# liruiw/OMG-Planner

Measured on AMD Instinct MI355X. Metric: CHOMP iterations/sec (batched scenes) + ms/plan, Panda 7-DoF 30-wp, higher is better.
Workload: dtype f32 SDF / f64 kinematics+update; 1 GPU; 100 table-top scenes/GPU x (64-goal goal-set cost + CHOMP step), Panda 9-dof, 30 waypoints; scenes_per_gpu=100, total_scenes=100, goals=64, waypoints=30, sdf_grid=4x64^3 + 128x96x32 per scene, private, goal_selection=MD on device (omgx_goal_update_optimize), pipeline_parts=3, top_k_collision=1000, plan_restart_every_steps=50

## Files before the change

### omg-planner_amd/csrc/omg_device.h

```cpp
#pragma once
#include <hip/hip_runtime.h>
#include <stdint.h>

#include "../../include/omg_hip.h"

#define OMG_WAVE 64

namespace omg {

struct __attribute__((packed, aligned(4))) F2 { float a, b; };
struct __attribute__((packed, aligned(4))) F4 { float a, b, c, d; };

__device__ __forceinline__ float lerpf(float a, float b, float t) { return __builtin_fmaf(t, b - a, a); }

struct Axis { int i0; float f; bool ok; };
__device__ __forceinline__ Axis axis_of(float g) {
    Axis a;
    a.ok = (g > -1.0e9f) && (g <= 1.0e9f);
    const float s = g - 0.5f;
    a.i0 = (int)s;
    a.f = s - (float)a.i0;
    const bool edge = (s == -1.0f) && (g > -0.5f);
    a.i0 = edge ? 0 : a.i0;
    a.f = edge ? -1.0f : a.f;
// ... 21 lines not shown
    const bool in = ax.ok && ay.ok && az.ok && ax.i0 >= 0 && ax.i0 < G.dx - 1 && ay.i0 >= 0 && ay.i0 < G.dy - 1 &&
                    az.i0 >= 0 && az.i0 < G.dz - 1;
    if (!in) return 1.0f;
    const int b = G.idx(ax.i0, ay.i0, az.i0);
    const int sy = G.dz, sx = G.dy * G.dz;
    const F2 r00 = *reinterpret_cast<const F2*>(G.g + b);
    const F2 r01 = *reinterpret_cast<const F2*>(G.g + b + sy);
    const F2 r10 = *reinterpret_cast<const F2*>(G.g + b + sx);
    const F2 r11 = *reinterpret_cast<const F2*>(G.g + b + sx + sy);
    return trilerp(r00.a, r00.b, r01.a, r01.b, r10.a, r10.b, r11.a, r11.b, ax.f, ay.f, az.f);
}

struct ObjParams {
    float T[12];
    float lo[3], hi[3];
    int dim[3];
    float delta, eps, pad, clr;
    double rw[3];
    float rc[3], rh[3], rr2;
    double rdelta;
    float i2eps, ieps;
};

__device__ __forceinline__ bool rbox_inside(float tx, float ty, float tz, const float* c, const float* h, float r2) {
    const float dx = __builtin_fmaxf(__builtin_fabsf(tx - c[0]) - h[0], 0.0f);
    const float dy = __builtin_fmaxf(__builtin_fabsf(ty - c[1]) - h[1], 0.0f);
    const float dz = __builtin_fmaxf(__builtin_fabsf(tz - c[2]) - h[2], 0.0f);
    return __builtin_fmaf(dz, dz, __builtin_fmaf(dy, dy, dx * dx)) <= r2;
}
__device__ __forceinline__ bool rbox_near(float ux, float uy, float uz, float rad, const float* c, const float* h, float r) {
    const float dx = __builtin_fmaxf(__builtin_fabsf(ux - c[0]) - h[0], 0.0f);
    const float dy = __builtin_fmaxf(__builtin_fabsf(uy - c[1]) - h[1], 0.0f);
    const float dz = __builtin_fmaxf(__builtin_fabsf(uz - c[2]) - h[2], 0.0f);
    const float rr = r + rad;
    return __builtin_fmaf(dz, dz, __builtin_fmaf(dy, dy, dx * dx)) <= rr * rr * 1.000001f;
}

__device__ __forceinline__ void derive_far_box(ObjParams& o) {
#pragma unroll
    for (int k = 0; k < 3; ++k) {
        const float w = o.hi[k] - o.lo[k];
        const bool ok = w > 0.0f && o.dim[k] > 0;
        const float vox = w / (float)(o.dim[k] > 0 ? o.dim[k] : 1);
        o.rc[k] = ok ? 0.5f * w : 0.0f;
        o.rh[k] = ok ? 0.5f * w + 1.5f * vox : __builtin_inff();
    }
    o.rr2 = 0.0f;
    o.rdelta = 1.0 / (double)o.delta;
    o.i2eps = 1.0f / (2.0f * o.eps);
    o.ieps = 1.0f / o.eps;
}

struct Accum { float pot, gx, gy, gz, col; };

struct PairPrep { float tx, ty, tz; bool far; };

__device__ __forceinline__ PairPrep pair_prepare(const ObjParams& o, float px, float py, float pz) {
    const float* T = o.T;
    const float ux = __builtin_fmaf(T[2], pz, __builtin_fmaf(T[1], py, __builtin_fmaf(T[0], px, T[3])));
    const float uy = __builtin_fmaf(T[6], pz, __builtin_fmaf(T[5], py, __builtin_fmaf(T[4], px, T[7])));
    const float uz = __builtin_fmaf(T[10], pz, __builtin_fmaf(T[9], py, __builtin_fmaf(T[8], px, T[11])));
    PairPrep r;
    r.tx = ux - o.lo[0]; r.ty = uy - o.lo[1]; r.tz = uz - o.lo[2];
    const bool inside = rbox_inside(r.tx, r.ty, r.tz, o.rc, o.rh, o.rr2);
    r.far = (o.eps < 1.0f && o.clr <= 1.0f) ? !inside : false;
    return r;
}

template <bool WANT_GRAD>
__device__ __forceinline__ void pair_exact(const ObjParams& o, const float* __restrict__ grid, float tx, float ty, float tz,
                                           Accum& acc) {
    const float* T = o.T;
    const float gx = (float)((double)tx * o.rw[0]) * (float)o.dim[0];
    const float gy = (float)((double)ty * o.rw[1]) * (float)o.dim[1];
    const float gz = (float)((double)tz * o.rw[2]) * (float)o.dim[2];
    Grid G{grid, o.dim[0], o.dim[1], o.dim[2]};
    const Axis ax = axis_of(gx), ay = axis_of(gy), az = axis_of(gz);
    const bool in_c = ax.ok && ay.ok && az.ok && ax.i0 >= 0 && ax.i0 < G.dx - 1 && ay.i0 >= 0 && ay.i0 < G.dy - 1 &&
                      az.i0 >= 0 && az.i0 < G.dz - 1;
    if (!in_c) {
        if (1.0f < o.clr) acc.col += 1.0f;
        if (!(1.0f <= o.eps)) return;
    }
    const int sy = G.dz, sx = G.dy * G.dz;
    const int b = G.idx(ax.i0, ay.i0, az.i0);

    if (!WANT_GRAD) {
        const int bb = in_c ? b : 0;
        const F2 r00 = *reinterpret_cast<const F2*>(G.g + bb);
        const F2 r01 = *reinterpret_cast<const F2*>(G.g + bb + sy);
        const F2 r10 = *reinterpret_cast<const F2*>(G.g + bb + sx);
        const F2 r11 = *reinterpret_cast<const F2*>(G.g + bb + sx + sy);
        const float tv = trilerp(r00.a, r00.b, r01.a, r01.b, r10.a, r10.b, r11.a, r11.b, ax.f, ay.f, az.f);
        const float value = in_c ? tv : 1.0f;
        acc.col += (in_c && value < o.clr) ? 1.0f : 0.0f;
        const float p_in = (float)(-(double)value + 0.5 * (double)o.eps);
        const float d = value - o.eps;
        const float p_band = o.i2eps * d * d * o.pad;
        acc.pot += value <= 0.0f ? p_in : (value <= o.eps ? p_band : 0.0f);
        return;
    }

    const Axis axp = axis_of(gx + 1.0f), axm = axis_of(gx - 1.0f);
    const Axis ayp = axis_of(gy + 1.0f), aym = axis_of(gy - 1.0f);
    const Axis azp = axis_of(gz + 1.0f), azm = axis_of(gz - 1.0f);
    const bool regular = axp.i0 == ax.i0 + 1 && axm.i0 == ax.i0 - 1 && ayp.i0 == ay.i0 + 1 && aym.i0 == ay.i0 - 1 &&
                         azp.i0 == az.i0 + 1 && azm.i0 == az.i0 - 1 && axp.ok && axm.ok && ayp.ok && aym.ok && azp.ok && azm.ok;
    const bool interior = in_c && regular && ax.i0 >= 1 && ax.i0 < G.dx - 2 && ay.i0 >= 1 && ay.i0 < G.dy - 2 &&
                          az.i0 >= 1 && az.i0 < G.dz - 2;

    float value, fpx, fmx, fpy, fmy, fpz, fmz;
    if (interior) {
        const F4 c00 = *reinterpret_cast<const F4*>(G.g + b - 1);
        const F4 c01 = *reinterpret_cast<const F4*>(G.g + b + sy - 1);
        const F4 c10 = *reinterpret_cast<const F4*>(G.g + b + sx - 1);
        const F4 c11 = *reinterpret_cast<const F4*>(G.g + b + sx + sy - 1);
        value = trilerp(c00.b, c00.c, c01.b, c01.c, c10.b, c10.c, c11.b, c11.c, ax.f, ay.f, az.f);
        if (value < o.clr) acc.col += 1.0f;
        if (!(value <= 0.0f || value <= o.eps)) return;
        fpz = trilerp(c00.c, c00.d, c01.c, c01.d, c10.c, c10.d, c11.c, c11.d, ax.f, ay.f, azp.f);
        fmz = trilerp(c00.a, c00.b, c01.a, c01.b, c10.a, c10.b, c11.a, c11.b, ax.f, ay.f, azm.f);
        const F2 xp0 = *reinterpret_cast<const F2*>(G.g + b + 2 * sx);
        const F2 xp1 = *reinterpret_cast<const F2*>(G.g + b + 2 * sx + sy);
        const F2 xm0 = *reinterpret_cast<const F2*>(G.g + b - sx);
        const F2 xm1 = *reinterpret_cast<const F2*>(G.g + b - sx + sy);
        fpx = trilerp(c10.b, c10.c, c11.b, c11.c, xp0.a, xp0.b, xp1.a, xp1.b, axp.f, ay.f, az.f);
        fmx = trilerp(xm0.a, xm0.b, xm1.a, xm1.b, c00.b, c00.c, c01.b, c01.c, axm.f, ay.f, az.f);
        const F2 yp0 = *reinterpret_cast<const F2*>(G.g + b + 2 * sy);
        const F2 yp1 = *reinterpret_cast<const F2*>(G.g + b + sx + 2 * sy);
        const F2 ym0 = *reinterpret_cast<const F2*>(G.g + b - sy);
        const F2 ym1 = *reinterpret_cast<const F2*>(G.g + b + sx - sy);
        fpy = trilerp(c01.b, c01.c, yp0.a, yp0.b, c11.b, c11.c, yp1.a, yp1.b, ax.f, ayp.f, az.f);
        fmy = trilerp(ym0.a, ym0.b, c00.b, c00.c, ym1.a, ym1.b, c10.b, c10.c, ax.f, aym.f, az.f);
    } else {
        if (in_c) {
            value = sdf_value(G, ax, ay, az);
            if (value < o.clr) acc.col += 1.0f;
            if (!(value <= 0.0f || value <= o.eps)) return;
        } else {
            value = 1.0f;
        }
        fpx = sdf_value(G, axp, ay, az);
        fpy = sdf_value(G, ax, ayp, az);
        fpz = sdf_value(G, ax, ay, azp);
        fmx = sdf_value(G, axm, ay, az);
        fmy = sdf_value(G, ax, aym, az);
        fmz = sdf_value(G, ax, ay, azm);
    }
    const float g0 = (float)(0.5 * (double)(fpx - fmx) * o.rdelta);
    const float g1 = (float)(0.5 * (double)(fpy - fmy) * o.rdelta);
    const float g2 = (float)(0.5 * (double)(fpz - fmz) * o.rdelta);
    float v0, v1, v2;
    if (value <= 0.0f) {
        acc.pot += (float)(-(double)value + 0.5 * (double)o.eps);
        v0 = -g0; v1 = -g1; v2 = -g2;
    } else {
        const float d = value - o.eps;
        acc.pot += o.i2eps * d * d * o.pad;
        const float ie = o.ieps;
        v0 = ie * g0 * d * o.pad; v1 = ie * g1 * d * o.pad; v2 = ie * g2 * d * o.pad;
    }
    acc.gx += __builtin_fmaf(T[8], v2, __builtin_fmaf(T[4], v1, T[0] * v0));
    acc.gy += __builtin_fmaf(T[9], v2, __builtin_fmaf(T[5], v1, T[1] * v0));
    acc.gz += __builtin_fmaf(T[10], v2, __builtin_fmaf(T[6], v1, T[2] * v0));
}

template <bool WANT_GRAD>
__device__ __forceinline__ void sdf_pair(const ObjParams& o, const float* __restrict__ grid, float px, float py, float pz,
                                         Accum& acc) {
    const PairPrep pp = pair_prepare(o, px, py, pz);
    if (!pp.far) pair_exact<WANT_GRAD>(o, grid, pp.tx, pp.ty, pp.tz, acc);
}

#define OMG_CONST_AS __attribute__((address_space(4)))
typedef const OMG_CONST_AS omgx_object* ObjTablePtr;
typedef const OMG_CONST_AS int32_t* IntTablePtr;
#define OMG_GLOBAL_AS __attribute__((address_space(1)))
typedef const OMG_GLOBAL_AS char* GlobalBytes;
typedef float F2v __attribute__((ext_vector_type(2), aligned(4)));
__device__ __forceinline__ F2 global_f2(GlobalBytes p) { const F2v v = *(const OMG_GLOBAL_AS F2v*)p; return F2{v.x, v.y}; }
__device__ __forceinline__ ObjTablePtr as_const(const omgx_object* p) { return (ObjTablePtr)(uintptr_t)p; }
__device__ __forceinline__ IntTablePtr as_const(const int32_t* p) { return (IntTablePtr)(uintptr_t)p; }

__device__ __forceinline__ ObjParams load_object(ObjTablePtr ob) {
    ObjParams o;
#pragma unroll
    for (int k = 0; k < 12; ++k) o.T[k] = ob->pose_inv[k];
#pragma unroll
    for (int k = 0; k < 3; ++k) { o.lo[k] = ob->lo[k]; o.hi[k] = ob->hi[k]; o.dim[k] = ob->dim[k]; }
// ... 290 lines not shown
```

### omg-planner_amd/csrc/omg_goalset_queue.h

```cpp
#pragma once

#define GQ_TBL_MAX 32
#ifndef GQ_WG_PER_CU
#define GQ_WG_PER_CU 5
#endif
#ifndef GQ_WAVES
#define GQ_WAVES 4
#endif
#define GQ_NT (64 * GQ_WAVES)

struct GqFar {
    float T[12], lo[3], rc[3], rh[3], rr2, rb_r;
    bool cullable;
    int disabled;
};

typedef uint32_t GqU16 __attribute__((ext_vector_type(16)));
typedef uint32_t GqU8 __attribute__((ext_vector_type(8)));
typedef uint32_t GqU4 __attribute__((ext_vector_type(4)));
static_assert(offsetof(omgx_object, pose_inv) == 0 && offsetof(omgx_object, lo) == 0x30 && offsetof(omgx_object, epsilon) == 0x58 &&
              offsetof(omgx_object, clearance) == 0x60 && offsetof(omgx_object, disabled) == 0x64 && offsetof(omgx_object, rb_c) == 0x88 &&
              offsetof(omgx_object, rb_h) == 0x94 && offsetof(omgx_object, rb_r) == 0xa0 && offsetof(omgx_object, rb_r2) == 0xa4 &&
              sizeof(omgx_object) >= 0xa8, "gq_load_far reads the record by byte offsets");
__device__ __forceinline__ GqFar gq_load_far(ObjTablePtr ob) {
// ... 66 lines not shown
}
__device__ __forceinline__ void gq_tbl_store(uint32_t* e, const GqTblRec& r) {
#pragma unroll
    for (int k = 0; k < 3; ++k) {
        e[2 * k] = (uint32_t)__double2loint(r.rw[k]); e[2 * k + 1] = (uint32_t)__double2hiint(r.rw[k]);
        e[6 + k] = (uint32_t)r.dim[k];
    }
    e[9] = (uint32_t)(r.goffb & 0xffffffffll); e[10] = (uint32_t)(r.goffb >> 32);
    e[11] = __float_as_uint(0.5f * r.eps);
    e[12] = __float_as_uint(r.eps); e[13] = __float_as_uint(r.clr);
    e[14] = __float_as_uint(r.pad); e[15] = __float_as_uint(r.i2e);
}

template <bool PERSIST>
__device__ __forceinline__ double gq_ld_traj(const double* p) {
    if constexpr (PERSIST) return __hip_atomic_load(p, __ATOMIC_RELAXED, __HIP_MEMORY_SCOPE_AGENT);
    else return *p;
}
template <bool PERSIST>
__device__ __forceinline__ void gq_st_out(float* p, float v) {
    if constexpr (PERSIST) __hip_atomic_store(p, v, __ATOMIC_RELAXED, __HIP_MEMORY_SCOPE_AGENT);
    else *p = v;
}

template <int LB, bool STAMP, bool LAT, bool SPLIT, bool PRE, bool PERSIST = false, int ROLE = 0, int W = GQ_WAVES, bool RANGE = false>
__device__ __forceinline__ void gq_item(const ChunkArgs& a, double* const lds_pose, const int s, const bool is_layer, const int layer_part, const int chunk, const int NP) {
    const int o_begin = as_const(a.scene_begin)[s], o_end = as_const(a.scene_begin)[s + 1];
    const int P = a.P;
    const bool warming = LAT && o_end > o_begin;
    const int goal = NP > 1 ? chunk / NP : chunk;
    const int part = NP > 1 ? chunk - goal * NP : 0;
    static_assert(!RANGE || (SPLIT && !LAT && !PRE && !PERSIST && W == GQ_WAVES), "waypoint ranges: the batch kernel with two parts per goal and their own kinematics");
    const int CHg = a.CH;
    const int cfg_off = (RANGE && part > 0) ? a.range_h : 0;
    const int CH = RANGE ? (part > 0 ? CHg - a.range_h : a.range_h) : CHg;
    const int blk_shift = (4 - (CH & 3)) & 3;
    const int p = threadIdx.x & 15, lane = threadIdx.x & 63;
    const int wave = __builtin_amdgcn_readfirstlane((int)(threadIdx.x >> 6));
    const int tid = (int)threadIdx.x;
    const RobotViewS rv(a.robot, P);
    const int pstride = a.PS, MR = a.MR;
    static_assert(W == GQ_WAVES || (!LAT && !SPLIT && !PRE && !PERSIST && W >= 4), "wide workgroups: the batch kernel with whole goals and its own kinematics");
    constexpr int NT = 64 * W;
    const GqLayout L(pstride, MR, P, a.tbl_n, LAT, W);
    char* const lds_bytes = reinterpret_cast<char*>(lds_pose);
    uint32_t* const rowmask = reinterpret_cast<uint32_t*>(lds_bytes + L.mask_off);
    uint32_t* const tilebits = reinterpret_cast<uint32_t*>(lds_bytes + L.tile_off);
    if (ROLE == 1 || (ROLE == 0 && is_layer)) {
        const int lgi = a.layer_nb > 1 ? layer_part / a.layer_nb : layer_part, cbi = layer_part - lgi * a.layer_nb;
        const int lpg = 10 / a.layer_lg, c_begin = cbi * a.layer_cb;
        const int c_end = c_begin + a.layer_cb < a.wp_n ? c_begin + a.layer_cb : a.wp_n;
        waypoint_layer_block<LAT, PERSIST>(a, s, lgi * lpg, (lgi + 1) * lpg, c_begin, c_end, lds_pose, rowmask, o_begin, o_end, rv,
                                  reinterpret_cast<double*>(lds_bytes + L.fkc_off), warming,
                                  reinterpret_cast<float*>(lds_bytes + L.objc_off), reinterpret_cast<double*>(lds_bytes + L.btab_off));
        GS_WG_STAMP(4);
        return;
    }
    if (a.goal_count && goal >= as_const(a.goal_count)[s]) {
        if (STAMP && tid == 0) a.work[(int64_t)s * a.NCH + chunk] = 0u;
        return;
    }
    const unsigned long long work_t0 = STAMP ? wall_clock64() : 0ull;
    GS_FREQ_BEGIN();
    uint32_t* const tbl = reinterpret_cast<uint32_t*>(lds_bytes + L.tbl_off);
    double* const pts = reinterpret_cast<double*>(lds_bytes + L.pts_off);
    float* const stage = reinterpret_cast<float*>(lds_bytes + L.stage_off) + wave * 256;

    auto cull_row = [&](int l, int ci) {
        const double* A = lds_pose + 9 + ((int64_t)l * pstride + ci) * 9;
        const auto bl = rv.ball(l);
        float cx, cy, cz;
        link_ball_center(A, A + 3, A + 6, bl, cx, cy, cz);
        const float rad = (float)bl[3] + 1.0e-4f;
        uint32_t m = 0;
        for (int o = o_begin; o < o_end; ++o) {
            ObjTablePtr ob = as_const(a.objects) + o;
            const GqFar f = gq_load_far(ob);
            if (f.disabled > 0) continue;
            const int oo = o - o_begin;
            const uint32_t bit = 1u << (oo < 31 ? oo : 31);
            float ux, uy, uz;
            se3_apply_s(f.T, cx, cy, cz, ux, uy, uz);
            const bool near = rbox_near(ux - f.lo[0], uy - f.lo[1], uz - f.lo[2], rad, f.rc, f.rh, f.rb_r);
            if (near || !f.cullable) m |= bit;
        }
        rowmask[l * CH + ci] = m;
        return m;
    };
    constexpr bool TILEBITS = !LAT && (!SPLIT || RANGE) && !PRE && LB == 2;
    const bool tb_on = TILEBITS;
    const bool tb_wide = CH > 32;
    auto tile_bit_set = [&](int rb, int pr) -> bool {
        if (!tb_wide) return (tilebits[pr >> 2] >> ((4 * rb + (pr & 3)) & 31)) & 1u;
        return pr < 4 ? ((tilebits[rb >> 3] >> (4 * (rb & 7) + pr)) & 1u) : ((tilebits[3] >> rb) & 1u);
    };
    if (tid < 4) tilebits[tid] = (tb_on || tid >= 2) ? 0u : 0xffffffffu;
    auto lat_tile = [&](int q) {
        const int ntl = ((CH + 3) >> 2) * (10 / LB);
        const int ntp = ntl > part ? (ntl - part + NP - 1) / NP : 0;
        const int r = 4 * q + ((q & 1) ? 3 - wave : wave);
        return r < ntp ? part + NP * (ntp - 1 - r) : -1;
    };
#ifndef OMGX_GS_BTAB_IN_PLACE
#define OMGX_GS_BTAB_IN_PLACE 1
#endif
    constexpr bool BTAB = !LAT && OMGX_GS_BTAB_IN_PLACE != 0;
    const int chain_waves = BTAB ? (CH + 1 + 20) / 21 : (3 * (CH + 1) + 63) >> 6;
// ... 444 lines not shown
                        GS_COUNT(7);
                        enqueue(live, live_mask, tx, ty, tz, w[k], (uint32_t)oo | (soft << 16));
                    } else if (live) {
                        ObjParams op = load_object(ob);
                        asm volatile("" : "+s"(op.eps), "+s"(op.clr));
                        Accum one{0.0f, 0.0f, 0.0f, 0.0f, 0.0f};
                        pair_exact<false>(op, h_pool + ob->grid_offset, tx, ty, tz, one);
                        if (soft) { one.pot *= 0.1f; one.col = 0.0f; }
                        add_term(one.pot != 0.0f ? one.pot * w[k] : 0.0f);
                        tcol += one.col;
                    }
                }
            }
        }
    }
    if (inflight) consume();
    if (pending > 0) {
        __builtin_amdgcn_fence(__ATOMIC_RELEASE, "wavefront");
        __builtin_amdgcn_wave_barrier();
        __builtin_amdgcn_fence(__ATOMIC_ACQUIRE, "wavefront");
        issue(pending);
        consume();
    }
#if defined(OMGX_GS_CLOCK)
    if (lane == 0 && blockIdx.x < (1u << 16)) {
        const unsigned long long now = wall_clock64();
        atomicMin(&g_gs_wg[GS_WG_IDX][5], now);
        atomicMax(&g_gs_wg[GS_WG_IDX][6], now);
    }
#endif
    {
        const double ws_ = wave_sum(tsum);
        const float wc_ = wave_sum(tcol);
        double* red = reinterpret_cast<double*>(lds_bytes + L.tbl_off);
        float* redc = reinterpret_cast<float*>(red + W);
        __syncthreads();
        if (lane == 0) { red[wave] = ws_; redc[wave] = wc_; }
        __syncthreads();
        if (tid == 0) {
            const int64_t k = (int64_t)s * a.NCH + chunk;
            double rs = ((red[0] + red[1]) + red[2]) + red[3];
            float rc = ((redc[0] + redc[1]) + redc[2]) + redc[3];
#pragma unroll
            for (int w = 4; w < W; ++w) { rs += red[w]; rc += redc[w]; }
            if (a.chunk_cost) gq_st_out<PERSIST>(a.chunk_cost + k, (float)rs);
            if (a.chunk_col) gq_st_out<PERSIST>(a.chunk_col + k, rc);
            if (STAMP) { const unsigned long long dt = wall_clock64() - work_t0; a.work[k] = dt < 1 ? 1u : (dt > 0xffffffffull ? 0xffffffffu : (uint32_t)dt); }
        }
    }
    GS_FREQ_END();
    GS_WG_STAMP(4);
}

template <int W> struct GqWide { static constexpr int wg_per_cu = W == GQ_WAVES ? GQ_WG_PER_CU : (W <= 6 ? 3 : 2); };
template <int LB, bool STAMP, bool LAT, bool SPLIT, bool PRE, int W, bool RANGE>
__device__ __forceinline__ void goalset_queue_body(const ChunkArgs& a, double* const lds_pose) {
    GS_WG_STAMP(0);
#ifdef OMGX_GS_PRIO
    __builtin_amdgcn_s_setprio(OMGX_GS_PRIO);
#endif
    const int xcd = blockIdx.x & 7;
    const int LPARTS = a.layer_parts;
    const bool spread = LAT;
    static_assert(!(LAT && SPLIT), "latency mode has its parts already");
    const int NP = (LAT || SPLIT) ? a.NP : 1;
    bool is_layer;
    int s, chunk, layer_part;
    bool scheduled = false;
    if (spread) {
        const int nl = a.wp_traj ? a.S * LPARTS : 0;
        is_layer = (int)blockIdx.x < nl;
        const int j = (int)blockIdx.x - nl;
        s = is_layer ? (int)blockIdx.x / LPARTS : j / a.NCH;
        layer_part = (int)blockIdx.x - s * LPARTS;
        chunk = is_layer ? 0 : j - s * a.NCH;
    } else {
        const int nlayer = a.wp_traj ? ((a.S + 7) >> 3) * LPARTS : 0;
        is_layer = (int)(blockIdx.x >> 3) < nlayer;
        const int j = (int)(blockIdx.x >> 3) - nlayer;
        const int sgrp = is_layer ? (int)(blockIdx.x >> 3) / LPARTS : j / a.NCH;
        layer_part = (int)(blockIdx.x >> 3) - sgrp * LPARTS;
        s = sgrp * 8 + xcd;
        chunk = is_layer ? 0 : j - sgrp * a.NCH;
        scheduled = a.schedule && !is_layer;
        if (scheduled) {
            const int item = as_const(a.schedule)[(int)blockIdx.x - nlayer * 8];
            if (item < 0 || item >= a.S * a.NCH) return;
            s = item / a.NCH;
            chunk = item - s * a.NCH;
            if (a.active && as_const(a.active)[s] == 0) { if (STAMP && threadIdx.x == 0) a.work[item] = 0u; return; }
        }
    }
    if (s >= a.S) return;
    if (a.active && !scheduled && !spread) {
        const int k = s, ln = threadIdx.x & 63;
        int seen = 0;
        s = -1;
        for (int base = 0; base < a.S; base += 64) {
            const int i = base + ln;
            const unsigned long long bal = __ballot(i < a.S && a.active[i] != 0);
            const int cnt = __popcll(bal);
            if (k < seen + cnt) {
                unsigned long long m = bal;
                for (int q = k - seen; q > 0; --q) m &= m - 1;
                s = base + __builtin_ctzll(m);
                break;
            }
            seen += cnt;
        }
    }
    if (s < 0) return;
    if (spread && a.active && as_const(a.active)[s] == 0) return;
    if constexpr (W != GQ_WAVES) {
        if (is_layer && threadIdx.x >= 64 * GQ_WAVES) return;
    }
    gq_item<LB, STAMP, LAT, SPLIT, PRE, false, 0, W, RANGE>(a, lds_pose, s, is_layer, layer_part, chunk, NP);
}

template <int LB, bool STAMP = false, bool LAT = false, bool SPLIT = false, bool PRE = false, int W = GQ_WAVES>
__global__ __launch_bounds__(LAT ? 256 : 64 * W, LAT ? 2 : GqWide<W>::wg_per_cu) void k_goalset_queue(ChunkArgs a) {
    extern __shared__ __attribute__((aligned(16))) double lds_pose[];
    goalset_queue_body<LB, STAMP, LAT, SPLIT, PRE, W, false>(a, lds_pose);
}

template <int LB, bool STAMP = false>
__global__ __launch_bounds__(GQ_NT, GQ_WG_PER_CU) void k_goalset_range(ChunkArgs a) {
    extern __shared__ __attribute__((aligned(16))) double lds_pose[];
    goalset_queue_body<LB, STAMP, false, true, false, GQ_WAVES, true>(a, lds_pose);
}
```

### omg-planner_amd/csrc/omg_kernels.hip

```cpp
#include <hip/hip_runtime.h>
#include <hip/hip_ext.h>

#include <stdint.h>
#include <stdio.h>
#include <stdlib.h>
#include <string.h>

#include <mutex>

#include "omg_device.h"
#include "omg_host.h"

using namespace omg;

struct RawObjects {
    const float* __restrict__ pose_init;
    const float* __restrict__ sdf_grids;
    const float* __restrict__ sdf_limits;
    const float* __restrict__ eps;
    const float* __restrict__ pad;
    const float* __restrict__ clr;
    const float* __restrict__ dis;
};

// ... 243 lines not shown
                        const float* grid = a.pool + ob->grid_offset;
                        PairPrep pp[LB];
#pragma unroll
                        for (int k = 0; k < LB; ++k) {
                            pp[k] = pair_prepare(op, px[k], py[k], pz[k]);
                            pp[k].far = pp[k].far || !(msk[k] & bit);
                        }
#pragma unroll
                        for (int k = 0; k < LB; ++k)
                            if (!pp[k].far) pair_exact<WANT_GRAD>(op, grid, pp[k].tx, pp[k].ty, pp[k].tz, acc[k]);
                    }
                }
#pragma unroll
                for (int k = 0; k < LB; ++k) {
                    const int l = l0 + k;
                    if (a.soften && l >= 8) {
                        acc[k].pot *= 0.1f; acc[k].gx *= 0.1f; acc[k].gy *= 0.1f; acc[k].gz *= 0.1f; acc[k].col = 0.0f;
                    }
                    if (a.arc && acc[k].pot != 0.0f) {
                        float qx, qy, qz;
                        pose12_apply(ci > 0 ? base + ((int64_t)l * pstride + ci - 1) * 12 : sbase + (int64_t)l * sstride, rv.pts(l, p), qx, qy, qz);
                        const float vx = (px[k] - qx) * a.inv_dt, vy = (py[k] - qy) * a.inv_dt, vz = (pz[k] - qz) * a.inv_dt;
                        acc[k].pot = acc[k].pot * sqrtf(vx * vx + vy * vy + vz * vz);
                    }
                    const int64_t kk = (out_cfg + l) * P + p;
                    if (a.pot) a.pot[kk] = acc[k].pot;
                    if (a.col) a.col[kk] = acc[k].col;
                    if (WANT_GRAD) { a.grad[3 * kk] = acc[k].gx; a.grad[3 * kk + 1] = acc[k].gy; a.grad[3 * kk + 2] = acc[k].gz; }
                    tsum += acc[k].pot;
                    tcol += acc[k].col;
                }
            }
        }
    }
    if (a.chunk_cost || a.chunk_col) {
        const float ws_ = wave_sum(tsum), wc_ = wave_sum(tcol);
        const int w = threadIdx.x >> 6;
        if ((threadIdx.x & 63) == 0) { red[0][w] = ws_; red[1][w] = wc_; }
        __syncthreads();
        if (threadIdx.x == 0) {
            const int64_t k = (int64_t)s * a.NCH + chunk;
            float c0 = red[0][0], c1 = red[1][0];
#pragma unroll
            for (int w2 = 1; w2 < TPB / 64; ++w2) { c0 += red[0][w2]; c1 += red[1][w2]; }
            if (a.chunk_cost) a.chunk_cost[k] = c0;
            if (a.chunk_col) a.chunk_col[k] = c1;
        }
    }
}
template <bool LAT, bool PERSIST = false>
__device__ __forceinline__ void waypoint_layer_block(const ChunkArgs& a, const int s, const int l_begin, const int l_end,
                                                     const int c_begin, const int c_end, double* lds_pose, uint32_t* rowmask,
                                                     const int o_begin, const int o_end, const RobotViewS& rv, double* fkc,
                                                     const bool warming, float* objc, double* btab) {
    const int n = a.wp_n, P = a.P, PS = a.PS, MR = a.MR;
    const int nloc = c_end - c_begin;
    const double* tr = a.wp_traj + ((int64_t)s * n + c_begin) * 9;
    double* sc = reinterpret_cast<double*>(rowmask);
    auto ldtr = [&](int k) -> double {
        if constexpr (PERSIST) return __hip_atomic_load(tr + k, __ATOMIC_RELAXED, __HIP_MEMORY_SCOPE_AGENT);
        else return tr[k];
    };
    const double fkv = (LAT && threadIdx.x < 246) ? rv.g[threadIdx.x] : 0.0;
    if (warming) gq_warm_scalar_cache(a.objects, o_begin, o_end, a.robot + OMGX_ROBOT_POINTS + 30 * P + 316 + 30 * P);
    for (int t = threadIdx.x; t < nloc * 7; t += 256) {
        const int cfg = t / 7, i = t - cfg * 7;
        double sn, cs;
        fk_joint_sincos(ldtr(cfg * 9 + i), sn, cs);
        sc[2 * t] = sn; sc[2 * t + 1] = cs;
    }
    if (LAT && threadIdx.x < 246) fkc[threadIdx.x] = fkv;
    __syncthreads();
    double* const gpose = (a.wp_pose_out && l_begin == 0) ? a.wp_pose_out + ((int64_t)s * n + c_begin) * 120 : nullptr;
    auto run_chain = [&](const auto& view) {
        for (int t = threadIdx.x; t < nloc * 3; t += 256) {
            const int cfg = t / 3, r = t - cfg * 3;
            fk_chain_row(view, r, sc + 14 * cfg, ldtr(cfg * 9 + 7), ldtr(cfg * 9 + 8), [&](int l, double r0, double r1, double r2, double tt) {
                double* dst = lds_pose + ((size_t)l * PS + cfg) * 9;
                if (r < 2) { dst[3 * r] = r0; dst[3 * r + 1] = r1; dst[3 * r + 2] = r2; }
                dst[6 + r] = tt;
                if (gpose) {
                    double* g = gpose + ((size_t)cfg * 10 + l) * 12;
                    g[3 * r] = r0; g[3 * r + 1] = r1; g[3 * r + 2] = r2; g[9 + r] = tt;
                }
            });
        }
    };
    if constexpr (LAT) {
        const RobotView rvl(a.robot, P, fkc);
        for (int t = threadIdx.x; t < nloc * 7; t += 256) fk_joint_matrix(rvl, t - (t / 7) * 7, sc[2 * t], sc[2 * t + 1], btab + 9 * t);
        __syncthreads();
        for (int t = threadIdx.x; t < nloc * 3; t += 256) {
            const int cfg = t / 3, r = t - cfg * 3;
            fk_chain_row_B(rvl, r, btab + 63 * cfg, ldtr(cfg * 9 + 7), ldtr(cfg * 9 + 8), [&](int l, double r0, double r1, double r2, double tt) {
                double* dst = lds_pose + ((size_t)l * PS + cfg) * 9;
                if (r < 2) { dst[3 * r] = r0; dst[3 * r + 1] = r1; dst[3 * r + 2] = r2; }
                dst[6 + r] = tt;
                if (gpose) {
                    double* g = gpose + ((size_t)cfg * 10 + l) * 12;
                    g[3 * r] = r0; g[3 * r + 1] = r1; g[3 * r + 2] = r2; g[9 + r] = tt;
                }
            });
        }
    } else run_chain(rv);
    __syncthreads();
    for (int row = l_begin * nloc + threadIdx.x; row < l_end * nloc; row += 256) {
        const int l = row / nloc, ci = row - l * nloc;
// ... 18 lines not shown
        }
        rowmask[l * MR + ci] = m;
    }
    __syncthreads();
    if (LAT && nloc <= 4 && l_end - l_begin == 1) {
        const int l = l_begin, lane = threadIdx.x & 63, wave = threadIdx.x >> 6;
        const int p = lane & 15, ci = lane >> 4;
        const bool valid = (p < P) && (ci < nloc);
        const int cic = valid ? ci : 0, pc = valid ? p : 0;
        const uint32_t msk = valid ? rowmask[l * MR + cic] : 0u;
        Accum acc{0.0f, 0.0f, 0.0f, 0.0f, 0.0f};
        if (__any(msk != 0)) {
            float px, py, pz;
            pose9_apply(lds_pose + ((int64_t)l * PS + cic) * 9, rv.pts(l, pc), px, py, pz);
            for (int og = o_begin; og < o_end; og += 8) {
                for (int o = og + wave; o < og + 8 && o < o_end; o += 4) {
                    const int oo = o - o_begin;
                    const uint32_t bit = 1u << (oo < 31 ? oo : 31);
                    Accum c{0.0f, 0.0f, 0.0f, 0.0f, 0.0f};
                    if (__any((msk & bit) != 0)) {
                        ObjTablePtr ob = as_const(a.objects) + o;
                        if (!(ob->disabled > 0)) {
                            const ObjParams op = load_object(ob);
                            const PairPrep pp = pair_prepare(op, px, py, pz);
                            if ((msk & bit) && !pp.far) pair_exact<true>(op, a.pool + ob->grid_offset, pp.tx, pp.ty, pp.tz, c);
                        }
                    }
                    float* dst = objc + ((o - og) * 64 + lane) * 5;
                    dst[0] = c.pot; dst[1] = c.gx; dst[2] = c.gy; dst[3] = c.gz; dst[4] = c.col;
                }
                __syncthreads();
                if (wave == 0) {
                    for (int o = og; o < og + 8 && o < o_end; ++o) {
                        const float* src = objc + ((o - og) * 64 + lane) * 5;
                        acc.pot += src[0]; acc.gx += src[1]; acc.gy += src[2]; acc.gz += src[3]; acc.col += src[4];
                    }
                }
                __syncthreads();
            }
        }
        if (wave == 0) {
            if (a.wp_soften && l >= 8) {
                acc.pot *= 0.1f; acc.gx *= 0.1f; acc.gy *= 0.1f; acc.gz *= 0.1f; acc.col = 0.0f;
            }
            if (valid) {
                const int64_t kk = (((int64_t)s * n + c_begin + ci) * 10 + l) * P + p;
                a.wp_pot[kk] = acc.pot;
                a.wp_col[kk] = acc.col;
                a.wp_grad[3 * kk] = acc.gx; a.wp_grad[3 * kk + 1] = acc.gy; a.wp_grad[3 * kk + 2] = acc.gz;
            }
        }
        return;
    }
    const int p = threadIdx.x & 15, r = threadIdx.x >> 4;
    for (int ci0 = 0; ci0 < nloc; ci0 += 16) {
        const int ci = ci0 + r;
        const bool valid = (p < P) && (ci < nloc);
        const int cic = valid ? ci : 0, pc = valid ? p : 0;
#pragma unroll 1
        for (int l = l_begin; l < l_end; ++l) {
            const uint32_t msk = valid ? rowmask[l * MR + cic] : 0u;
            Accum acc{0.0f, 0.0f, 0.0f, 0.0f, 0.0f};
            if (__any(msk != 0)) {
                float px, py, pz;
                pose9_apply(lds_pose + ((int64_t)l * PS + cic) * 9, rv.pts(l, pc), px, py, pz);
                for (int o = o_begin; o < o_end; ++o) {
                    const int oo = o - o_begin;
                    const uint32_t bit = 1u << (oo < 31 ? oo : 31);
                    if (!__any((msk & bit) != 0)) continue;
                    ObjTablePtr ob = as_const(a.objects) + o;
                    if (ob->disabled > 0) continue;
                    const ObjParams op = load_object(ob);
                    const PairPrep pp = pair_prepare(op, px, py, pz);
                    if ((msk & bit) && !pp.far) pair_exact<true>(op, a.pool + ob->grid_offset, pp.tx, pp.ty, pp.tz, acc);
                }
            }
            if (a.wp_soften && l >= 8) {
                acc.pot *= 0.1f; acc.gx *= 0.1f; acc.gy *= 0.1f; acc.gz *= 0.1f; acc.col = 0.0f;
            }
            if (valid) {
                const int64_t kk = (((int64_t)s * n + c_begin + ci) * 10 + l) * P + p;
                a.wp_pot[kk] = acc.pot;
                a.wp_col[kk] = acc.col;
                a.wp_grad[3 * kk] = acc.gx; a.wp_grad[3 * kk + 1] = acc.gy; a.wp_grad[3 * kk + 2] = acc.gz;
            }
        }
    }
}

#ifdef OMGX_GS_CLOCK
__device__ unsigned long long g_gs_wg[1 << 16][8];
#define GS_WG_IDX ((blockIdx.x + (((unsigned)a.S & 1u) << 14)) & 0xffffu)
#define GS_WG_STAMP(k) do { if (threadIdx.x == 0 && blockIdx.x < (1u << 16)) { g_gs_wg[GS_WG_IDX][k] = wall_clock64(); if (k == 0) { g_gs_wg[GS_WG_IDX][5] = ~0ull; g_gs_wg[GS_WG_IDX][6] = 0ull; unsigned hw, xcc; asm volatile("s_getreg_b32 %0, hwreg(HW_REG_HW_ID)" : "=s"(hw)); asm volatile("s_getreg_b32 %0, hwreg(HW_REG_XCC_ID)" : "=s"(xcc)); g_gs_wg[GS_WG_IDX][7] = ((unsigned long long)xcc << 32) | hw; } } } while (0)
__device__ unsigned long long g_gs_wave[1 << 16][8];
#define GS_WAVE_STAMP(k) do { if ((threadIdx.x & 63) == 0 && (k) < 8 && blockIdx.x < (1u << 16)) g_gs_wave[blockIdx.x][k] = wall_clock64(); } while (0)
extern "C" int omgx_debug_gs_wave(unsigned long long* h_out, int n_wg) {
    if (n_wg > (1 << 16)) n_wg = 1 << 16;
    return hipMemcpyFromSymbol(h_out, HIP_SYMBOL(g_gs_wave), sizeof(unsigned long long) * 8 * n_wg) == hipSuccess ? 0 : -2;
}
__device__ unsigned long long g_gs_freq[1 << 16][2];
#define GS_FREQ_BEGIN() unsigned long long gs_f0 = 0, gs_f1 = 0; if (threadIdx.x == 0) { gs_f0 = __builtin_readcyclecounter(); gs_f1 = wall_clock64(); }
#define GS_FREQ_END() do { if (threadIdx.x == 0 && blockIdx.x < (1u << 16)) { g_gs_freq[blockIdx.x][0] = __builtin_readcyclecounter() - gs_f0; g_gs_freq[blockIdx.x][1] = wall_clock64() - gs_f1; } } while (0)
extern "C" int omgx_debug_gs_freq(unsigned long long* h_out, int n_wg) {
    if (n_wg > (1 << 16)) n_wg = 1 << 16;
    return hipMemcpyFromSymbol(h_out, HIP_SYMBOL(g_gs_freq), sizeof(unsigned long long) * 2 * n_wg) == hipSuccess ? 0 : -2;
}
extern "C" int omgx_debug_gs_wg(unsigned long long* h_out, int n_wg) {
    if (n_wg > (1 << 16)) n_wg = 1 << 16;
    return hipMemcpyFromSymbol(h_out, HIP_SYMBOL(g_gs_wg), sizeof(unsigned long long) * 8 * n_wg) == hipSuccess ? 0 : -2;
}
#else
#define GS_WG_STAMP(k)
#define GS_WAVE_STAMP(k)
#define GS_FREQ_BEGIN()
#define GS_FREQ_END()
#endif

#if defined(OMGX_GS_ADD_S)
#define GS_MARGINAL_COST_PROBE(a_, b_, c_, d_, i_, j_) do { { uint32_t d0 = (uint32_t)(i_), d1 = (uint32_t)(j_); asm volatile("s_add_u32 %0, %0, 3\n\ts_add_u32 %1, %1, 5\n\ts_add_u32 %0, %0, 3\n\ts_add_u32 %1, %1, 5\n\ts_add_u32 %0, %0, 3\n\ts_add_u32 %1, %1, 5\n\ts_add_u32 %0, %0, 3\n\ts_add_u32 %1, %1, 5\n\t" "s_add_u32 %0, %0, 3\n\ts_add_u32 %1, %1, 5\n\ts_add_u32 %0, %0, 3\n\ts_add_u32 %1, %1, 5\n\ts_add_u32 %0, %0, 3\n\ts_add_u32 %1, %1, 5\n\ts_add_u32 %0, %0, 3\n\ts_add_u32 %1, %1, 5" : "+s"(d0), "+s"(d1) : : "scc"); } } while (0)
#elif defined(OMGX_GS_ADD_V)
#define GS_MARGINAL_COST_PROBE(a_, b_, c_, d_, i_, j_) do { { float d0 = (a_), d1 = (b_), d2 = (c_), d3 = (d_); asm volatile("v_fma_f32 %0, %0, %0, %0\n\tv_fma_f32 %1, %1, %1, %1\n\tv_fma_f32 %2, %2, %2, %2\n\tv_fma_f32 %3, %3, %3, %3\n\t" "v_fma_f32 %0, %0, %0, %0\n\tv_fma_f32 %1, %1, %1, %1\n\tv_fma_f32 %2, %2, %2, %2\n\tv_fma_f32 %3, %3, %3, %3\n\t" "v_fma_f32 %0, %0, %0, %0\n\tv_fma_f32 %1, %1, %1, %1\n\tv_fma_f32 %2, %2, %2, %2\n\tv_fma_f32 %3, %3, %3, %3\n\t" "v_fma_f32 %0, %0, %0, %0\n\tv_fma_f32 %1, %1, %1, %1\n\tv_fma_f32 %2, %2, %2, %2\n\tv_fma_f32 %3, %3, %3, %3" : "+v"(d0), "+v"(d1), "+v"(d2), "+v"(d3)); } } while (0)
#elif defined(OMGX_GS_ADD_V64)
#define GS_MARGINAL_COST_PROBE(a_, b_, c_, d_, i_, j_) do { { double d0 = (a_), d1 = (b_), d2 = (c_), d3 = (d_); asm volatile("v_fma_f64 %0, %0, %0, %0\n\tv_fma_f64 %1, %1, %1, %1\n\tv_fma_f64 %2, %2, %2, %2\n\tv_fma_f64 %3, %3, %3, %3\n\t" "v_fma_f64 %0, %0, %0, %0\n\tv_fma_f64 %1, %1, %1, %1\n\tv_fma_f64 %2, %2, %2, %2\n\tv_fma_f64 %3, %3, %3, %3\n\t" "v_fma_f64 %0, %0, %0, %0\n\tv_fma_f64 %1, %1, %1, %1\n\tv_fma_f64 %2, %2, %2, %2\n\tv_fma_f64 %3, %3, %3, %3\n\t" "v_fma_f64 %0, %0, %0, %0\n\tv_fma_f64 %1, %1, %1, %1\n\tv_fma_f64 %2, %2, %2, %2\n\tv_fma_f64 %3, %3, %3, %3" : "+v"(d0), "+v"(d1), "+v"(d2), "+v"(d3)); } } while (0)
#elif defined(OMGX_GS_ADD_B)
#define GS_MARGINAL_COST_PROBE(a_, b_, c_, d_, i_, j_) do { asm volatile("s_branch 1f\n\ts_nop 0\n\t1:\n\ts_branch 2f\n\ts_nop 0\n\t2:\n\ts_branch 3f\n\ts_nop 0\n\t3:\n\ts_branch 4f\n\ts_nop 0\n\t4:\n\t" "s_branch 5f\n\ts_nop 0\n\t5:\n\ts_branch 6f\n\ts_nop 0\n\t6:\n\ts_branch 7f\n\ts_nop 0\n\t7:\n\ts_branch 8f\n\ts_nop 0\n\t8:"); } while (0)
#elif defined(OMGX_GS_ADD_N)
#define GS_MARGINAL_COST_PROBE(a_, b_, c_, d_, i_, j_) do { asm volatile("s_nop 0\n\ts_nop 0\n\ts_nop 0\n\ts_nop 0\n\ts_nop 0\n\ts_nop 0\n\ts_nop 0\n\ts_nop 0\n\ts_nop 0\n\ts_nop 0\n\ts_nop 0\n\ts_nop 0\n\ts_nop 0\n\ts_nop 0\n\ts_nop 0\n\ts_nop 0"); } while (0)
#else
#define GS_MARGINAL_COST_PROBE(a_, b_, c_, d_, i_, j_) do { } while (0)
#endif

#ifdef OMGX_GS_COUNT
__device__ unsigned long long g_gs_count[16];
#define GS_COUNT(k) do { if ((threadIdx.x & 63) == 0) atomicAdd(&g_gs_count[k], 1ull); } while (0)
#define GS_COUNT_N(k, n) do { const unsigned long long n_ = (unsigned long long)(n); if ((threadIdx.x & 63) == 0) atomicAdd(&g_gs_count[k], n_); } while (0)
extern "C" int omgx_debug_gs_counts(unsigned long long* h_out, int reset) {
    if (hipMemcpyFromSymbol(h_out, HIP_SYMBOL(g_gs_count), sizeof(unsigned long long) * 16) != hipSuccess) return -2;
// ... 912 lines not shown
```

Before: 552,100 iterations/s.

## Software-pipeline SDF centre loads across live objects in waypoint layer block

The per-point object loop is split into two phases. A first pass builds live and wave-live object masks. A second pass then issues the centre-cell grid loads for the next live object before consuming the current one, so memory latency overlaps with trilinear work. Accumulators are moved to an LDS staging slot, and the lane index is recomputed behind asm barriers to cut register pressure. The launch-bounds occupancy value for the wide variant is also changed. The cost is recomputing the transform and cell setup several times per object, plus extra LDS traffic for the accumulators.

```diff
diff --git a/omg-planner_amd/csrc/omg_device.h b/omg-planner_amd/csrc/omg_device.h
--- a/omg-planner_amd/csrc/omg_device.h
+++ b/omg-planner_amd/csrc/omg_device.h
@@ -97,6 +97,7 @@
 }
 
 struct Accum { float pot, gx, gy, gz, col; };
+struct AccumRef { float& pot; float& gx; float& gy; float& gz; float& col; };
 
 struct PairPrep { float tx, ty, tz; bool far; };
 
@@ -112,17 +113,64 @@
     return r;
 }
 
-template <bool WANT_GRAD>
+struct PairCell { float gx, gy, gz; Axis ax, ay, az; bool in_c; };
+__device__ __forceinline__ PairCell pair_cell(const ObjParams& o, float tx, float ty, float tz) {
+    PairCell c;
+    c.gx = (float)((double)tx * o.rw[0]) * (float)o.dim[0];
+    c.gy = (float)((double)ty * o.rw[1]) * (float)o.dim[1];
+    c.gz = (float)((double)tz * o.rw[2]) * (float)o.dim[2];
+    c.ax = axis_of(c.gx); c.ay = axis_of(c.gy); c.az = axis_of(c.gz);
+    c.in_c = c.ax.ok && c.ay.ok && c.az.ok && c.ax.i0 >= 0 && c.ax.i0 < o.dim[0] - 1 && c.ay.i0 >= 0 && c.ay.i0 < o.dim[1] - 1 &&
+             c.az.i0 >= 0 && c.az.i0 < o.dim[2] - 1;
+    return c;
+}
+struct PairShift { Axis axp, axm, ayp, aym, azp, azm; bool interior; };
+__device__ __forceinline__ PairShift pair_shift(const ObjParams& o, const PairCell& c) {
+    PairShift s;
+    s.axp = axis_of(c.gx + 1.0f); s.axm = axis_of(c.gx - 1.0f);
+    s.ayp = axis_of(c.gy + 1.0f); s.aym = axis_of(c.gy - 1.0f);
+    s.azp = axis_of(c.gz + 1.0f); s.azm = axis_of(c.gz - 1.0f);
+    const bool regular = s.axp.i0 == c.ax.i0 + 1 && s.axm.i0 == c.ax.i0 - 1 && s.ayp.i0 == c.ay.i0 + 1 && s.aym.i0 == c.ay.i0 - 1 &&
+                         s.azp.i0 == c.az.i0 + 1 && s.azm.i0 == c.az.i0 - 1 && s.axp.ok && s.axm.ok && s.ayp.ok && s.aym.ok && s.azp.ok && s.azm.ok;
+    s.interior = c.in_c && regular && c.ax.i0 >= 1 && c.ax.i0 < o.dim[0] - 2 && c.ay.i0 >= 1 && c.ay.i0 < o.dim[1] - 2 &&
+                 c.az.i0 >= 1 && c.az.i0 < o.dim[2] - 2;
+    return s;
+}
+template <typename ROW>
+__device__ __forceinline__ ROW grid_row(const float* __restrict__ g, uint32_t byte_off) {
+    return *reinterpret_cast<const ROW*>(reinterpret_cast<const char*>(g) + byte_off);
+}
+struct CentreRows { F4 c00, c01, c10, c11; };
+__device__ __forceinline__ CentreRows pair_centre_rows(const float* __restrict__ g, uint32_t b4, uint32_t sx4, uint32_t sy4) {
+    CentreRows r;
+    r.c00 = grid_row<F4>(g, b4 - 4u);
+    r.c01 = grid_row<F4>(g, b4 + sy4 - 4u);
+    r.c10 = grid_row<F4>(g, b4 + sx4 - 4u);
+    r.c11 = grid_row<F4>(g, b4 + sx4 + sy4 - 4u);
+    return r;
+}
+struct CentreMid { F2 m00, m01, m10, m11; };
+__device__ __forceinline__ CentreMid pair_issue_centre(const ObjParams& o, const float* __restrict__ grid, float tx, float ty, float tz, bool live) {
+    const PairCell c = pair_cell(o, tx, ty, tz);
+    const Grid G{grid, o.dim[0], o.dim[1], o.dim[2]};
+    const bool want = live && c.in_c;
+    const uint32_t b4 = want ? 4u * (uint32_t)G.idx(c.ax.i0, c.ay.i0, c.az.i0) : 0u, sy4 = 4u * (uint32_t)G.dz, sx4 = 4u * (uint32_t)(G.dy * G.dz);
+    CentreMid r;
+    r.m00 = grid_row<F2>(grid, b4);
+    r.m01 = grid_row<F2>(grid, b4 + sy4);
+    r.m10 = grid_row<F2>(grid, b4 + sx4);
+    r.m11 = grid_row<F2>(grid, b4 + sx4 + sy4);
+    return r;
+}
+
+template <bool WANT_GRAD, bool PRE = false, class ACC = Accum>
 __device__ __forceinline__ void pair_exact(const ObjParams& o, const float* __restrict__ grid, float tx, float ty, float tz,
-                                           Accum& acc) {
+                                           ACC& acc, const CentreMid& pre = CentreMid{}) {
     const float* T = o.T;
-    const float gx = (float)((double)tx * o.rw[0]) * (float)o.dim[0];
-    const float gy = (float)((double)ty * o.rw[1]) * (float)o.dim[1];
-    const float gz = (float)((double)tz * o.rw[2]) * (float)o.dim[2];
+    const PairCell pc = pair_cell(o, tx, ty, tz);
     Grid G{grid, o.dim[0], o.dim[1], o.dim[2]};
-    const Axis ax = axis_of(gx), ay = axis_of(gy), az = axis_of(gz);
-    const bool in_c = ax.ok && ay.ok && az.ok && ax.i0 >= 0 && ax.i0 < G.dx - 1 && ay.i0 >= 0 && ay.i0 < G.dy - 1 &&
-                      az.i0 >= 0 && az.i0 < G.dz - 1;
+    const Axis ax = pc.ax, ay = pc.ay, az = pc.az;
+    const bool in_c = pc.in_c;
     if (!in_c) {
         if (1.0f < o.clr) acc.col += 1.0f;
         if (!(1.0f <= o.eps)) return;
@@ -146,40 +194,39 @@
         return;
     }
 
-    const Axis axp = axis_of(gx + 1.0f), axm = axis_of(gx - 1.0f);
-    const Axis ayp = axis_of(gy + 1.0f), aym = axis_of(gy - 1.0f);
-    const Axis azp = axis_of(gz + 1.0f), azm = axis_of(gz - 1.0f);
-    const bool regular = axp.i0 == ax.i0 + 1 && axm.i0 == ax.i0 - 1 && ayp.i0 == ay.i0 + 1 && aym.i0 == ay.i0 - 1 &&
-                         azp.i0 == az.i0 + 1 && azm.i0 == az.i0 - 1 && axp.ok && axm.ok && ayp.ok && aym.ok && azp.ok && azm.ok;
-    const bool interior = in_c && regular && ax.i0 >= 1 && ax.i0 < G.dx - 2 && ay.i0 >= 1 && ay.i0 < G.dy - 2 &&
-                          az.i0 >= 1 && az.i0 < G.dz - 2;
+    const PairShift ps = pair_shift(o, pc);
+    const Axis axp = ps.axp, axm = ps.axm, ayp = ps.ayp, aym = ps.aym, azp = ps.azp, azm = ps.azm;
+    const bool interior = ps.interior;
 
     float value, fpx, fmx, fpy, fmy, fpz, fmz;
     if (interior) {
-        const F4 c00 = *reinterpret_cast<const F4*>(G.g + b - 1);
-        const F4 c01 = *reinterpret_cast<const F4*>(G.g + b + sy - 1);
-        const F4 c10 = *reinterpret_cast<const F4*>(G.g + b + sx - 1);
-        const F4 c11 = *reinterpret_cast<const F4*>(G.g + b + sx + sy - 1);
-        value = trilerp(c00.b, c00.c, c01.b, c01.c, c10.b, c10.c, c11.b, c11.c, ax.f, ay.f, az.f);
+        const uint32_t b4 = 4u * (uint32_t)b, sx4 = 4u * (uint32_t)sx, sy4 = 4u * (uint32_t)sy;
+        CentreRows cr;
+        if (!PRE) cr = pair_centre_rows(G.g, b4, sx4, sy4);
+        value = PRE ? trilerp(pre.m00.a, pre.m00.b, pre.m01.a, pre.m01.b, pre.m10.a, pre.m10.b, pre.m11.a, pre.m11.b, ax.f, ay.f, az.f)
+                    : trilerp(cr.c00.b, cr.c00.c, cr.c01.b, cr.c01.c, cr.c10.b, cr.c10.c, cr.c11.b, cr.c11.c, ax.f, ay.f, az.f);
         if (value < o.clr) acc.col += 1.0f;
         if (!(value <= 0.0f || value <= o.eps)) return;
+        if (PRE) cr = pair_centre_rows(G.g, b4, sx4, sy4);
+        const F4 c00 = cr.c00, c01 = cr.c01, c10 = cr.c10, c11 = cr.c11;
         fpz = trilerp(c00.c, c00.d, c01.c, c01.d, c10.c, c10.d, c11.c, c11.d, ax.f, ay.f, azp.f);
         fmz = trilerp(c00.a, c00.b, c01.a, c01.b, c10.a, c10.b, c11.a, c11.b, ax.f, ay.f, azm.f);
-        const F2 xp0 = *reinterpret_cast<const F2*>(G.g + b + 2 * sx);
-        const F2 xp1 = *reinterpret_cast<const F2*>(G.g + b + 2 * sx + sy);
-        const F2 xm0 = *reinterpret_cast<const F2*>(G.g + b - sx);
-        const F2 xm1 = *reinterpret_cast<const F2*>(G.g + b - sx + sy);
+        const F2 xp0 = grid_row<F2>(G.g, b4 + 2u * sx4);
+        const F2 xp1 = grid_row<F2>(G.g, b4 + 2u * sx4 + sy4);
+        const F2 xm0 = grid_row<F2>(G.g, b4 - sx4);
+        const F2 xm1 = grid_row<F2>(G.g, b4 - sx4 + sy4);
         fpx = trilerp(c10.b, c10.c, c11.b, c11.c, xp0.a, xp0.b, xp1.a, xp1.b, axp.f, ay.f, az.f);
         fmx = trilerp(xm0.a, xm0.b, xm1.a, xm1.b, c00.b, c00.c, c01.b, c01.c, axm.f, ay.f, az.f);
-        const F2 yp0 = *reinterpret_cast<const F2*>(G.g + b + 2 * sy);
-        const F2 yp1 = *reinterpret_cast<const F2*>(G.g + b + sx + 2 * sy);
-        const F2 ym0 = *reinterpret_cast<const F2*>(G.g + b - sy);
-        const F2 ym1 = *reinterpret_cast<const F2*>(G.g + b + sx - sy);
+        const F2 yp0 = grid_row<F2>(G.g, b4 + 2u * sy4);
+        const F2 yp1 = grid_row<F2>(G.g, b4 + sx4 + 2u * sy4);
+        const F2 ym0 = grid_row<F2>(G.g, b4 - sy4);
+        const F2 ym1 = grid_row<F2>(G.g, b4 + sx4 - sy4);
         fpy = trilerp(c01.b, c01.c, yp0.a, yp0.b, c11.b, c11.c, yp1.a, yp1.b, ax.f, ayp.f, az.f);
         fmy = trilerp(ym0.a, ym0.b, c00.b, c00.c, ym1.a, ym1.b, c10.b, c10.c, ax.f, aym.f, az.f);
     } else {
         if (in_c) {
-            value = sdf_value(G, ax, ay, az);
+            value = PRE ? trilerp(pre.m00.a, pre.m00.b, pre.m01.a, pre.m01.b, pre.m10.a, pre.m10.b, pre.m11.a, pre.m11.b, ax.f, ay.f, az.f)
+                        : sdf_value(G, ax, ay, az);
             if (value < o.clr) acc.col += 1.0f;
             if (!(value <= 0.0f || value <= o.eps)) return;
         } else {
diff --git a/omg-planner_amd/csrc/omg_goalset_queue.h b/omg-planner_amd/csrc/omg_goalset_queue.h
--- a/omg-planner_amd/csrc/omg_goalset_queue.h
+++ b/omg-planner_amd/csrc/omg_goalset_queue.h
@@ -142,7 +142,8 @@
         const int c_end = c_begin + a.layer_cb < a.wp_n ? c_begin + a.layer_cb : a.wp_n;
         waypoint_layer_block<LAT, PERSIST>(a, s, lgi * lpg, (lgi + 1) * lpg, c_begin, c_end, lds_pose, rowmask, o_begin, o_end, rv,
                                   reinterpret_cast<double*>(lds_bytes + L.fkc_off), warming,
-                                  reinterpret_cast<float*>(lds_bytes + L.objc_off), reinterpret_cast<double*>(lds_bytes + L.btab_off));
+                                  reinterpret_cast<float*>(lds_bytes + L.objc_off), reinterpret_cast<double*>(lds_bytes + L.btab_off),
+                                  reinterpret_cast<float*>(lds_bytes + L.stage_off));
         GS_WG_STAMP(4);
         return;
     }
@@ -693,7 +694,7 @@
     GS_WG_STAMP(4);
 }
 
-template <int W> struct GqWide { static constexpr int wg_per_cu = W == GQ_WAVES ? GQ_WG_PER_CU : (W <= 6 ? 3 : 2); };
+template <int W> struct GqWide { static constexpr int waves_per_simd = GQ_WG_PER_CU; };
 template <int LB, bool STAMP, bool LAT, bool SPLIT, bool PRE, int W, bool RANGE>
 __device__ __forceinline__ void goalset_queue_body(const ChunkArgs& a, double* const lds_pose) {
     GS_WG_STAMP(0);
@@ -759,7 +760,7 @@
 }
 
 template <int LB, bool STAMP = false, bool LAT = false, bool SPLIT = false, bool PRE = false, int W = GQ_WAVES>
-__global__ __launch_bounds__(LAT ? 256 : 64 * W, LAT ? 2 : GqWide<W>::wg_per_cu) void k_goalset_queue(ChunkArgs a) {
+__global__ __launch_bounds__(LAT ? 256 : 64 * W, LAT ? 2 : GqWide<W>::waves_per_simd) void k_goalset_queue(ChunkArgs a) {
     extern __shared__ __attribute__((aligned(16))) double lds_pose[];
     goalset_queue_body<LB, STAMP, LAT, SPLIT, PRE, W, false>(a, lds_pose);
 }
diff --git a/omg-planner_amd/csrc/omg_kernels.hip b/omg-planner_amd/csrc/omg_kernels.hip
--- a/omg-planner_amd/csrc/omg_kernels.hip
+++ b/omg-planner_amd/csrc/omg_kernels.hip
@@ -319,7 +319,7 @@
 __device__ __forceinline__ void waypoint_layer_block(const ChunkArgs& a, const int s, const int l_begin, const int l_end,
                                                      const int c_begin, const int c_end, double* lds_pose, uint32_t* rowmask,
                                                      const int o_begin, const int o_end, const RobotViewS& rv, double* fkc,
-                                                     const bool warming, float* objc, double* btab) {
+                                                     const bool warming, float* objc, double* btab, float* accs) {
     const int n = a.wp_n, P = a.P, PS = a.PS, MR = a.MR;
     const int nloc = c_end - c_begin;
     const double* tr = a.wp_traj + ((int64_t)s * n + c_begin) * 9;
@@ -444,37 +444,93 @@
         }
         return;
     }
-    const int p = threadIdx.x & 15, r = threadIdx.x >> 4;
+    auto lane_of = [&](int ci0, int& p, int& ci) {
+        unsigned t = threadIdx.x;
+        asm volatile("" : "+v"(t));
+        p = (int)(t & 15u); ci = ci0 + (int)(t >> 4);
+        return (p < P) && (ci < nloc);
+    };
     for (int ci0 = 0; ci0 < nloc; ci0 += 16) {
-        const int ci = ci0 + r;
-        const bool valid = (p < P) && (ci < nloc);
-        const int cic = valid ? ci : 0, pc = valid ? p : 0;
 #pragma unroll 1
         for (int l = l_begin; l < l_end; ++l) {
-            const uint32_t msk = valid ? rowmask[l * MR + cic] : 0u;
-            Accum acc{0.0f, 0.0f, 0.0f, 0.0f, 0.0f};
+            int p0, ci_0;
+            const bool valid0 = lane_of(ci0, p0, ci_0);
+            const int cic = valid0 ? ci_0 : 0, pc = valid0 ? p0 : 0;
+            const uint32_t msk = valid0 ? rowmask[l * MR + cic] : 0u;
+            float* const slot = accs + 4 * threadIdx.x;
+            float col = 0.0f;
+            asm volatile("" : "+v"(col));
+            slot[0] = col; slot[1] = col; slot[2] = col; slot[3] = col;
+            AccumRef acc{slot[0], slot[1], slot[2], slot[3], col};
             if (__any(msk != 0)) {
                 float px, py, pz;
                 pose9_apply(lds_pose + ((int64_t)l * PS + cic) * 9, rv.pts(l, pc), px, py, pz);
-                for (int o = o_begin; o < o_end; ++o) {
-                    const int oo = o - o_begin;
-                    const uint32_t bit = 1u << (oo < 31 ? oo : 31);
+                const int n_own = o_end - o_begin < 31 ? o_end - o_begin : 31;
+                uint32_t lm = msk & (1u << 31), wm = 0u;
+                for (int oo = 0; oo < n_own; ++oo) {
+                    const uint32_t bit = 1u << oo;
                     if (!__any((msk & bit) != 0)) continue;
-                    ObjTablePtr ob = as_const(a.objects) + o;
+                    ObjTablePtr ob = as_const(a.objects) + o_begin + oo;
                     if (ob->disabled > 0) continue;
                     const ObjParams op = load_object(ob);
+                    const bool live = (msk & bit) && !pair_prepare(op, px, py, pz).far;
+                    lm |= live ? bit : 0u;
+                    wm |= __builtin_amdgcn_ballot_w64(live) != 0ull ? bit : 0u;
+                }
+                auto issue = [&](int oo) -> CentreMid {
+                    ObjTablePtr ob = as_const(a.objects) + o_begin + oo;
+                    const ObjParams op = load_object(ob);
                     const PairPrep pp = pair_prepare(op, px, py, pz);
-                    if ((msk & bit) && !pp.far) pair_exact<true>(op, a.pool + ob->grid_offset, pp.tx, pp.ty, pp.tz, acc);
+                    return pair_issue_centre(op, a.pool + ob->grid_offset, pp.tx, pp.ty, pp.tz, (lm >> oo) & 1u);
+                };
+                auto consume = [&](int oo, const CentreMid& rows) {
+                    float qx = px, qy = py, qz = pz;
+                    asm volatile("" : "+v"(qx), "+v"(qy), "+v"(qz) : : "memory");
+                    asm volatile("" : "+s"(oo));
+                    ObjTablePtr ob = as_const(a.objects) + o_begin + oo;
+                    const ObjParams op = load_object(ob);
+                    const PairPrep pp = pair_prepare(op, qx, qy, qz);
+                    if ((lm >> oo) & 1u) pair_exact<true, true>(op, a.pool + ob->grid_offset, pp.tx, pp.ty, pp.tz, acc, rows);
+                };
+                auto next_live = [&]() { const int oo = __builtin_ctz(wm); wm &= wm - 1u; return oo; };
+                if (wm != 0u) {
+                    int ka = next_live(), kb = 0;
+                    CentreMid ra = issue(ka), rb{};
+                    bool last_a;
+                    for (;;) {
+                        if (wm == 0u) { last_a = true; break; }
+                        kb = next_live(); rb = issue(kb);
+                        consume(ka, ra);
+                        if (wm == 0u) { last_a = false; break; }
+                        ka = next_live(); ra = issue(ka);
+                        consume(kb, rb);
+                    }
+                    if (last_a) consume(ka, ra); else consume(kb, rb);
+                }
+                if (__any((lm >> 31) != 0u)) {
+                    for (int o = o_begin + 31; o < o_end; ++o) {
+                        ObjTablePtr ob = as_const(a.objects) + o;
+                        if (ob->disabled > 0) continue;
+                        const ObjParams op = load_object(ob);
+                        const PairPrep pp = pair_prepare(op, px, py, pz);
+                        const bool live = (lm >> 31) && !pp.far;
+                        if (__builtin_amdgcn_ballot_w64(live) == 0ull) continue;
+                        const float* grid = a.pool + ob->grid_offset;
+                        const CentreMid rows = pair_issue_centre(op, grid, pp.tx, pp.ty, pp.tz, live);
+                        if (live) pair_exact<true, true>(op, grid, pp.tx, pp.ty, pp.tz, acc, rows);
+                    }
                 }
             }
+            Accum sum{slot[0], slot[1], slot[2], slot[3], col};
             if (a.wp_soften && l >= 8) {
-                acc.pot *= 0.1f; acc.gx *= 0.1f; acc.gy *= 0.1f; acc.gz *= 0.1f; acc.col = 0.0f;
+                sum.pot *= 0.1f; sum.gx *= 0.1f; sum.gy *= 0.1f; sum.gz *= 0.1f; sum.col = 0.0f;
             }
-            if (valid) {
+            int p, ci;
+            if (lane_of(ci0, p, ci)) {
                 const int64_t kk = (((int64_t)s * n + c_begin + ci) * 10 + l) * P + p;
-                a.wp_pot[kk] = acc.pot;
-                a.wp_col[kk] = acc.col;
-                a.wp_grad[3 * kk] = acc.gx; a.wp_grad[3 * kk + 1] = acc.gy; a.wp_grad[3 * kk + 2] = acc.gz;
+                a.wp_pot[kk] = sum.pot;
+                a.wp_col[kk] = sum.col;
+                a.wp_grad[3 * kk] = sum.gx; a.wp_grad[3 * kk + 1] = sum.gy; a.wp_grad[3 * kk + 2] = sum.gz;
             }
         }
     }
```

After: 545,700 iterations/s. -1.2%, worse.
